# the3cloud/zktls

Hardware: AMD Instinct MI355X
Metric: trace-cells/s (higher is better)
Workload: dtype u32

## Files before the change

### zktls_amd/csrc/hash.hip

```cpp
#include "poseidon2.cuh"
#include "poseidon2_coop.cuh"
#include "kernels.h"
#include "batch.h"
#include "p24chip.h"
#include "p24chip_rows.cuh"
#include "p2chip.h"

namespace zk {

hipError_t hash_upload_p2_tables(const P2Tables& t, hipStream_t s) { return p2_upload_tables(t, s); }

__device__ __forceinline__ uint32_t load_virtual(const LeafArgs& a, uint64_t row, uint32_t vc) {
    uint32_t off = vc;
#pragma unroll
    for (int m = 0; m < MAX_LEAF_MATS; m++) {
        if (m < a.nmats) {
            if (off < a.mats[m].width) return a.mats[m].ptr[row * a.mats[m].ld + off];
            off -= a.mats[m].width;
        }
    }
    return 0u;
}

__global__ void hash_rows16_kernel(LeafArgs a, uint32_t total_w);
struct hash_rows16_kernel_bargs { LeafArgs a; uint32_t total_w; static hash_rows16_kernel_bargs make(LeafArgs a, uint32_t total_w) { return hash_rows16_kernel_bargs{a, total_w}; } };
__global__ void hash_rows16_kernel_batch(const hash_rows16_kernel_bargs* __restrict__ zk_arr);
__global__ void compress_level16_kernel(const uint32_t* __restrict__ children, uint32_t* __restrict__ parents, uint32_t count);
struct compress_level16_kernel_bargs { const uint32_t* children; uint32_t* parents; uint32_t count; static compress_level16_kernel_bargs make(const uint32_t* children, uint32_t* parents, uint32_t count) { return compress_level16_kernel_bargs{children, parents, count}; } };
__global__ void compress_level16_kernel_batch(const compress_level16_kernel_bargs* __restrict__ zk_arr);
__global__ void compress_top16_kernel(uint32_t* tree, uint32_t count);
struct compress_top16_kernel_bargs { uint32_t* tree; uint32_t count; static compress_top16_kernel_bargs make(uint32_t* tree, uint32_t count) { return compress_top16_kernel_bargs{tree, count}; } };
__global__ void compress_top16_kernel_batch(const compress_top16_kernel_bargs* __restrict__ zk_arr);
__global__ void compress_sub16_kernel(uint32_t* tree, uint32_t count, uint32_t sub);
struct compress_sub16_kernel_bargs { uint32_t* tree; uint32_t count; uint32_t sub; static compress_sub16_kernel_bargs make(uint32_t* tree, uint32_t count, uint32_t sub) { return compress_sub16_kernel_bargs{tree, count, sub}; } };
__global__ void compress_sub16_kernel_batch(const compress_sub16_kernel_bargs* __restrict__ zk_arr);
__global__ void hash_sub16_kernel(LeafArgs a, uint32_t total_w, uint32_t sub);
struct hash_sub16_kernel_bargs { LeafArgs a; uint32_t total_w; uint32_t sub; static hash_sub16_kernel_bargs make(LeafArgs a, uint32_t total_w, uint32_t sub) { return hash_sub16_kernel_bargs{a, total_w, sub}; } };
__global__ void hash_sub16_kernel_batch(const hash_sub16_kernel_bargs* __restrict__ zk_arr);

__device__ __forceinline__ void hash_rows_generic_kernel_body(const LeafArgs& a, uint32_t total_w) {
    const uint64_t row = (uint64_t)blockIdx.x * blockDim.x + threadIdx.x;
    if (row >= a.height) return;
    uint32_t s[16];
#pragma unroll
    for (int i = 0; i < 16; i++) s[i] = 0u;
    for (uint32_t q = 0; q < total_w; q += 8) {
#pragma unroll
        for (int i = 0; i < 8; i++)
            if (q + i < total_w) s[i] = load_virtual(a, row, q + i);
        p2_permute_dev(s);
    }
    uint4* d = reinterpret_cast<uint4*>(a.digests + row * 8);
    d[0] = make_uint4(s[0], s[1], s[2], s[3]);
    d[1] = make_uint4(s[4], s[5], s[6], s[7]);
}
__global__ void __launch_bounds__(256) hash_rows_generic_kernel(LeafArgs a, uint32_t total_w) { hash_rows_generic_kernel_body(a, total_w); }
struct hash_rows_generic_kernel_bargs { LeafArgs a; uint32_t total_w; static hash_rows_generic_kernel_bargs make(LeafArgs a, uint32_t total_w) { return hash_rows_generic_kernel_bargs{a, total_w}; } };
__global__ void __launch_bounds__(256) hash_rows_generic_kernel_batch(const hash_rows_generic_kernel_bargs* __restrict__ zk_arr) { const hash_rows_generic_kernel_bargs& zk_b = zk_arr[blockIdx.z]; hash_rows_generic_kernel_body(zk_b.a, zk_b.total_w); }


template <bool MX>
__device__ __forceinline__ void hash_rows_vec_body(const uint32_t* __restrict__ mat, uint64_t ld, uint32_t width, uint64_t height, uint32_t* __restrict__ digests) {
    const uint64_t row = (uint64_t)blockIdx.x * blockDim.x + threadIdx.x;
    if (MX ? row - __lane_id() >= height : row >= height) return;
    const uint4* rp = reinterpret_cast<const uint4*>(mat + (row < height ? row : height - 1) * ld);
    uint32_t s[16];
#pragma unroll
    for (int i = 0; i < 16; i++) s[i] = 0u;
    for (uint32_t q = 0; q < width / 8; q++) {
        uint4 v0 = rp[2 * q], v1 = rp[2 * q + 1];
        s[0] = v0.x; s[1] = v0.y; s[2] = v0.z; s[3] = v0.w;
        s[4] = v1.x; s[5] = v1.y; s[6] = v1.z; s[7] = v1.w;
        if (MX) p2_permute_mx_dev(s); else p2_permute_dev(s);
    }
    if (width & 4u) {
        const uint4 v0 = rp[width / 4 - 1];
        s[0] = v0.x; s[1] = v0.y; s[2] = v0.z; s[3] = v0.w;
        if (MX) p2_permute_mx_dev(s); else p2_permute_dev(s);
    }
    if (row >= height) return;
    uint4* d = reinterpret_cast<uint4*>(digests + row * 8);
    d[0] = make_uint4(s[0], s[1], s[2], s[3]);
    d[1] = make_uint4(s[4], s[5], s[6], s[7]);
}
__device__ __forceinline__ void hash_rows_vec_kernel_body(const uint32_t* __restrict__ mat, uint64_t ld, uint32_t width, uint64_t height, uint32_t* __restrict__ digests) { hash_rows_vec_body<true>(mat, ld, width, height, digests); }
__global__ void __launch_bounds__(256) __attribute__((amdgpu_waves_per_eu(5))) hash_rows_vec_kernel(const uint32_t* __restrict__ mat, uint64_t ld, uint32_t width, uint64_t height, uint32_t* __restrict__ digests) { hash_rows_vec_kernel_body(mat, ld, width, height, digests); }
struct hash_rows_vec_kernel_bargs { const uint32_t* mat; uint64_t ld; uint32_t width; uint64_t height; uint32_t* digests; static hash_rows_vec_kernel_bargs make(const uint32_t* mat, uint64_t ld, uint32_t width, uint64_t height, uint32_t* digests) { return hash_rows_vec_kernel_bargs{mat, ld, width, height, digests}; } };
__global__ void __launch_bounds__(256) __attribute__((amdgpu_waves_per_eu(5))) hash_rows_vec_kernel_batch(const hash_rows_vec_kernel_bargs* __restrict__ zk_arr) { const hash_rows_vec_kernel_bargs& zk_b = zk_arr[blockIdx.z]; hash_rows_vec_kernel_body(zk_b.mat, zk_b.ld, zk_b.width, zk_b.height, zk_b.digests); }
#ifdef ZKHIP_AB_HOOKS
__global__ void __launch_bounds__(256) hash_rows_vec_valu_kernel(const uint32_t* __restrict__ mat, uint64_t ld, uint32_t width, uint64_t height, uint32_t* __restrict__ digests) { hash_rows_vec_body<false>(mat, ld, width, height, digests); }
#endif

__device__ __forceinline__ void sponge_rows_vec(const LeafArgs& a, uint64_t row, uint32_t total_q, uint32_t s[16]) {
    int m = 0;
    uint32_t q = 0, nq = a.mats[0].width / 4;
    const uint4* rp = reinterpret_cast<const uint4*>(a.mats[0].ptr + row * a.mats[0].ld);
    for (uint32_t b = 0; b < total_q; b += 2) {
        while (q == nq) { m++; q = 0; nq = a.mats[m].width / 4; rp = reinterpret_cast<const uint4*>(a.mats[m].ptr + row * a.mats[m].ld); }
        const uint4 v0 = rp[q++];
        s[0] = v0.x; s[1] = v0.y; s[2] = v0.z; s[3] = v0.w;
        if (b + 1 < total_q) {
            while (q == nq) { m++; q = 0; nq = a.mats[m].width / 4; rp = reinterpret_cast<const uint4*>(a.mats[m].ptr + row * a.mats[m].ld); }
            const uint4 v1 = rp[q++];
            s[4] = v1.x; s[5] = v1.y; s[6] = v1.z; s[7] = v1.w;
        }
        p2_permute_dev(s);
    }
}
__device__ __forceinline__ void hash_rows_mvec_kernel_body(const LeafArgs& a, uint32_t total_q) {
    const uint64_t row = (uint64_t)blockIdx.x * blockDim.x + threadIdx.x;
    if (row >= a.height) return;
    uint32_t s[16];
#pragma unroll
    for (int i = 0; i < 16; i++) s[i] = 0u;
    sponge_rows_vec(a, row, total_q, s);
    uint4* d = reinterpret_cast<uint4*>(a.digests + row * 8);
    d[0] = make_uint4(s[0], s[1], s[2], s[3]);
    d[1] = make_uint4(s[4], s[5], s[6], s[7]);
}
__global__ void __launch_bounds__(256) hash_rows_mvec_kernel(LeafArgs a, uint32_t total_q) { hash_rows_mvec_kernel_body(a, total_q); }
struct hash_rows_mvec_kernel_bargs { LeafArgs a; uint32_t total_q; static hash_rows_mvec_kernel_bargs make(LeafArgs a, uint32_t total_q) { return hash_rows_mvec_kernel_bargs{a, total_q}; } };
__global__ void __launch_bounds__(256) hash_rows_mvec_kernel_batch(const hash_rows_mvec_kernel_bargs* __restrict__ zk_arr) { const hash_rows_mvec_kernel_bargs& zk_b = zk_arr[blockIdx.z]; hash_rows_mvec_kernel_body(zk_b.a, zk_b.total_q); }

__device__ __forceinline__ void compress_inject_mvec_kernel_body(const uint32_t* __restrict__ children, const LeafArgs& a, uint32_t total_q) {
    const uint64_t i = (uint64_t)blockIdx.x * blockDim.x + threadIdx.x;
    if (i >= a.height) return;
    const uint4* cp = reinterpret_cast<const uint4*>(children + 16 * i);
    const uint4 c0 = cp[0], c1 = cp[1], c2 = cp[2], c3 = cp[3];
    uint32_t s[16] = {c0.x, c0.y, c0.z, c0.w, c1.x, c1.y, c1.z, c1.w, c2.x, c2.y, c2.z, c2.w, c3.x, c3.y, c3.z, c3.w};
    uint32_t t[16];
#pragma unroll
    for (int k = 0; k < 16; k++) t[k] = 0u;
    p2_permute_dev(s);
    sponge_rows_vec(a, i, total_q, t);
#pragma unroll
    for (int k = 0; k < 8; k++) s[8 + k] = t[k];
    p2_permute_dev(s);
    uint4* d = reinterpret_cast<uint4*>(a.digests + i * 8);
    d[0] = make_uint4(s[0], s[1], s[2], s[3]);
    d[1] = make_uint4(s[4], s[5], s[6], s[7]);
}
__global__ void __launch_bounds__(256) compress_inject_mvec_kernel(const uint32_t* __restrict__ children, LeafArgs a, uint32_t total_q) { compress_inject_mvec_kernel_body(children, a, total_q); }
struct compress_inject_mvec_kernel_bargs { const uint32_t* children; LeafArgs a; uint32_t total_q; static compress_inject_mvec_kernel_bargs make(const uint32_t* children, LeafArgs a, uint32_t total_q) { return compress_inject_mvec_kernel_bargs{children, a, total_q}; } };
__global__ void __launch_bounds__(256) compress_inject_mvec_kernel_batch(const compress_inject_mvec_kernel_bargs* __restrict__ zk_arr) { const compress_inject_mvec_kernel_bargs& zk_b = zk_arr[blockIdx.z]; compress_inject_mvec_kernel_body(zk_b.children, zk_b.a, zk_b.total_q); }

static bool leaf_mats_vec(const LeafArgs& a) {
    for (int m = 0; m < a.nmats; m++) {
        const MatDesc& d = a.mats[m];
        if (d.width == 0 || d.width % 4 || d.ld % 4 || (reinterpret_cast<uintptr_t>(d.ptr) & 15)) return false;
    }
    return a.nmats >= 1;
}
hipError_t launch_compress_inject(const uint32_t* children, const LeafArgs& a, hipStream_t s) {
    if (a.height == 0) return hipSuccess;
    if (a.nmats < 1 || a.nmats > MAX_LEAF_MATS || !leaf_mats_vec(a)) return hipErrorInvalidValue;
    uint32_t total = 0;
    for (int m = 0; m < a.nmats; m++) total += a.mats[m].width;
    ZK_LAUNCH(compress_inject_mvec_kernel, compress_inject_mvec_kernel_batch, compress_inject_mvec_kernel_bargs, dim3((unsigned)((a.height + 255) / 256)), dim3(256), 0, s, children, a, total / 4);
    return hipGetLastError();
}
bool compress_inject_ok(const LeafArgs& a) { return a.height > coop_max_nodes() && leaf_mats_vec(a); }

hipError_t launch_hash_rows(const LeafArgs& a, hipStream_t s) {
    if (a.height == 0) return hipSuccess;
    if (a.nmats < 1 || a.nmats > MAX_LEAF_MATS) return hipErrorInvalidValue;
    uint32_t total = 0;
    for (int m = 0; m < a.nmats; m++) total += a.mats[m].width;
    if (a.height <= coop_max_nodes()) {
        const uint64_t threads = a.height * 16;
        ZK_LAUNCH(hash_rows16_kernel, hash_rows16_kernel_batch, hash_rows16_kernel_bargs, dim3((unsigned)((threads + 255) / 256)), dim3(256), 0, s, a, total);
        return hipGetLastError();
    }
    dim3 block(256), grid((unsigned)((a.height + 255) / 256));
    const MatDesc& m0 = a.mats[0];
    bool vec = a.nmats == 1 && m0.width % 4 == 0 && m0.ld % 4 == 0 &&
               (reinterpret_cast<uintptr_t>(m0.ptr) & 15) == 0;
#ifdef ZKHIP_AB_HOOKS
    static const bool valu = getenv("ZKHIP_HASH_VEC_VALU") != nullptr;
    if (vec && valu) {
        hash_rows_vec_valu_kernel<<<grid, block, 0, s>>>(m0.ptr, m0.ld, m0.width, a.height, a.digests);
        return hipGetLastError();
    }
#endif
    if (vec)
        ZK_LAUNCH(hash_rows_vec_kernel, hash_rows_vec_kernel_batch, hash_rows_vec_kernel_bargs, grid, block, 0, s, m0.ptr, m0.ld, m0.width, a.height, a.digests);
    else if (leaf_mats_vec(a))
        ZK_LAUNCH(hash_rows_mvec_kernel, hash_rows_mvec_kernel_batch, hash_rows_mvec_kernel_bargs, grid, block, 0, s, a, total / 4);
    else
        ZK_LAUNCH(hash_rows_generic_kernel, hash_rows_generic_kernel_batch, hash_rows_generic_kernel_bargs, grid, block, 0, s, a, total);
    return hipGetLastError();
}

__device__ __forceinline__ void compress_node(const uint32_t* children, uint32_t* parent) {
    const uint4* cp = reinterpret_cast<const uint4*>(children);
    uint4 v0 = cp[0], v1 = cp[1], v2 = cp[2], v3 = cp[3];
    uint32_t s[16] = {v0.x, v0.y, v0.z, v0.w, v1.x, v1.y, v1.z, v1.w,
                      v2.x, v2.y, v2.z, v2.w, v3.x, v3.y, v3.z, v3.w};
    p2_permute_dev(s);
    uint4* d = reinterpret_cast<uint4*>(parent);
    d[0] = make_uint4(s[0], s[1], s[2], s[3]);
    d[1] = make_uint4(s[4], s[5], s[6], s[7]);
}

__device__ __forceinline__ void compress_level_kernel_body(const uint32_t* __restrict__ children, uint32_t* __restrict__ parents, uint64_t count) {
    const uint64_t i = (uint64_t)blockIdx.x * blockDim.x + threadIdx.x;
    if (i >= count) return;
    compress_node(children + 16 * i, parents + 8 * i);
}
__global__ void __launch_bounds__(256) compress_level_kernel(const uint32_t* __restrict__ children, uint32_t* __restrict__ parents, uint64_t count) { compress_level_kernel_body(children, parents, count); }
struct compress_level_kernel_bargs { const uint32_t* children; uint32_t* parents; uint64_t count; static compress_level_kernel_bargs make(const uint32_t* children, uint32_t* parents, uint64_t count) { return compress_level_kernel_bargs{children, parents, count}; } };
__global__ void __launch_bounds__(256) compress_level_kernel_batch(const compress_level_kernel_bargs* __restrict__ zk_arr) { const compress_level_kernel_bargs& zk_b = zk_arr[blockIdx.z]; compress_level_kernel_body(zk_b.children, zk_b.parents, zk_b.count); }

hipError_t launch_compress_level(const uint32_t* children, uint32_t* parents, uint64_t count, hipStream_t s) {
    if (count == 0) return hipSuccess;
    if (count <= coop_max_nodes()) {
        const uint64_t threads = count * 16;
        ZK_LAUNCH(compress_level16_kernel, compress_level16_kernel_batch, compress_level16_kernel_bargs, dim3((unsigned)((threads + 255) / 256)), dim3(256), 0, s, children, parents, (uint32_t)count);
        return hipGetLastError();
    }
    ZK_LAUNCH(compress_level_kernel, compress_level_kernel_batch, compress_level_kernel_bargs, dim3((unsigned)((count + 255) / 256)), dim3(256), 0, s, children, parents, count);
    return hipGetLastError();
}

__device__ __forceinline__ void inject_kernel_body(uint32_t* __restrict__ nodes, const uint32_t* __restrict__ extra, uint64_t count) {
    const uint64_t i = (uint64_t)blockIdx.x * blockDim.x + threadIdx.x;
    if (i >= count) return;
    const uint4* a = reinterpret_cast<const uint4*>(nodes + 8 * i);
    const uint4* b = reinterpret_cast<const uint4*>(extra + 8 * i);
    const uint4 v0 = a[0], v1 = a[1], v2 = b[0], v3 = b[1];
    uint32_t s[16] = {v0.x, v0.y, v0.z, v0.w, v1.x, v1.y, v1.z, v1.w, v2.x, v2.y, v2.z, v2.w, v3.x, v3.y, v3.z, v3.w};
    p2_permute_dev(s);
    uint4* d = reinterpret_cast<uint4*>(nodes + 8 * i);
    d[0] = make_uint4(s[0], s[1], s[2], s[3]);
    d[1] = make_uint4(s[4], s[5], s[6], s[7]);
}
__global__ void __launch_bounds__(256) inject_kernel(uint32_t* __restrict__ nodes, const uint32_t* __restrict__ extra, uint64_t count) { inject_kernel_body(nodes, extra, count); }
struct inject_kernel_bargs { uint32_t* nodes; const uint32_t* extra; uint64_t count; static inject_kernel_bargs make(uint32_t* nodes, const uint32_t* extra, uint64_t count) { return inject_kernel_bargs{nodes, extra, count}; } };
__global__ void __launch_bounds__(256) inject_kernel_batch(const inject_kernel_bargs* __restrict__ zk_arr) { const inject_kernel_bargs& zk_b = zk_arr[blockIdx.z]; inject_kernel_body(zk_b.nodes, zk_b.extra, zk_b.count); }

hipError_t launch_inject(uint32_t* nodes, const uint32_t* extra, uint64_t count, hipStream_t s) {
    if (count == 0) return hipSuccess;
    ZK_LAUNCH(inject_kernel, inject_kernel_batch, inject_kernel_bargs, dim3((unsigned)((count + 255) / 256)), dim3(256), 0, s, nodes, extra, count);
    return hipGetLastError();
}

__device__ __forceinline__ void compress_top_kernel_body(uint32_t* tree, uint32_t count) {
    uint32_t* level = tree;
    for (uint32_t n = count; n > 1; n >>= 1) {
        uint32_t* next = level + 8 * (size_t)n;
        for (uint32_t i = threadIdx.x; i < n / 2; i += blockDim.x) compress_node(level + 16 * (size_t)i, next + 8 * (size_t)i);
        __threadfence_block();
        __syncthreads();
        level = next;
    }
}
__global__ void __launch_bounds__(1024) compress_top_kernel(uint32_t* tree, uint32_t count) { compress_top_kernel_body(tree, count); }
struct compress_top_kernel_bargs { uint32_t* tree; uint32_t count; static compress_top_kernel_bargs make(uint32_t* tree, uint32_t count) { return compress_top_kernel_bargs{tree, count}; } };
__global__ void __launch_bounds__(1024) compress_top_kernel_batch(const compress_top_kernel_bargs* __restrict__ zk_arr) { const compress_top_kernel_bargs& zk_b = zk_arr[blockIdx.z]; compress_top_kernel_body(zk_b.tree, zk_b.count); }

hipError_t launch_compress_top(uint32_t* tree, uint32_t count, hipStream_t s) {
    if (count <= 1) return hipSuccess;
    if (count > COOP_TOP_NODES) return hipErrorInvalidValue;
    unsigned threads = count * 8 < 64 ? 64 : (count * 8 > 1024 ? 1024 : count * 8);
// ... 957 lines not shown
```

### zktls_amd/csrc/poseidon2.cuh

```cuda
#pragma once
#include "babybear.cuh"
#include "p2_params.h"

namespace zk {

struct P2Consts {
    uint32_t ext_rc[8][16];
    uint32_t int_rc[13];
    uint32_t diag[16];
    uint32_t ext_rcm[8][16];
    uint32_t int_rcm[13];
};
struct P2Raw {
    uint32_t ext16[8][16], int16[13], diag16[16];
    uint32_t ext24[8][24], int24[21], diag24[24];
};
constexpr P2Consts make_p2_consts(const P2Raw& raw) {
    P2Consts k{};
    for (int r = 0; r < 8; r++)
        for (int i = 0; i < 16; i++) k.ext_rc[r][i] = to_monty(raw.ext16[r][i]);
    for (int r = 0; r < 13; r++) k.int_rc[r] = to_monty(raw.int16[r]);
    for (int i = 0; i < 16; i++) k.diag[i] = to_monty(raw.diag16[i]);
    for (int r = 0; r < 8; r++)
        for (int i = 0; i < 16; i++) k.ext_rcm[r][i] = k.ext_rc[r][i] - P;
// ... 33 lines not shown
}

ZK_HD constexpr void p2_external_linear(uint32_t s[16]) {
    p2_m4(s[0], s[1], s[2], s[3]);
    p2_m4(s[4], s[5], s[6], s[7]);
    p2_m4(s[8], s[9], s[10], s[11]);
    p2_m4(s[12], s[13], s[14], s[15]);
    uint32_t t0 = fadd(fadd(s[0], s[4]), fadd(s[8], s[12]));
    uint32_t t1 = fadd(fadd(s[1], s[5]), fadd(s[9], s[13]));
    uint32_t t2 = fadd(fadd(s[2], s[6]), fadd(s[10], s[14]));
    uint32_t t3 = fadd(fadd(s[3], s[7]), fadd(s[11], s[15]));
#if defined(__HIP_DEVICE_COMPILE__)
#pragma unroll
#endif
    for (int b = 0; b < 16; b += 4) {
        s[b] = fadd(s[b], t0);
        s[b + 1] = fadd(s[b + 1], t1);
        s[b + 2] = fadd(s[b + 2], t2);
        s[b + 3] = fadd(s[b + 3], t3);
    }
}

struct Mat4 { uint32_t m[4][4]; };
template <bool HL>
constexpr Mat4 m4_matrix() {
    Mat4 a{};
    for (int j = 0; j < 4; j++) {
        uint32_t e[4] = {0, 0, 0, 0};
        e[j] = MONTY_R1;
        if (HL) p2_m4_hl(e[0], e[1], e[2], e[3]); else p2_m4(e[0], e[1], e[2], e[3]);
        for (int i = 0; i < 4; i++) a.m[i][j] = e[i];
    }
    return a;
}
constexpr Mat4 mat4_inverse(Mat4 a) {
    Mat4 b{};
    for (int i = 0; i < 4; i++) b.m[i][i] = MONTY_R1;
    for (int c = 0; c < 4; c++) {
        int piv = c;
        while (a.m[piv][c] == 0) piv++;
        for (int j = 0; j < 4; j++) {
            uint32_t t = a.m[c][j]; a.m[c][j] = a.m[piv][j]; a.m[piv][j] = t;
            t = b.m[c][j]; b.m[c][j] = b.m[piv][j]; b.m[piv][j] = t;
        }
        const uint32_t inv = finv(a.m[c][c]);
        for (int j = 0; j < 4; j++) { a.m[c][j] = fmul(a.m[c][j], inv); b.m[c][j] = fmul(b.m[c][j], inv); }
        for (int r = 0; r < 4; r++) {
            if (r == c) continue;
            const uint32_t f = a.m[r][c];
            for (int j = 0; j < 4; j++) {
                a.m[r][j] = fsub(a.m[r][j], fmul(f, a.m[c][j]));
                b.m[r][j] = fsub(b.m[r][j], fmul(f, b.m[c][j]));
            }
        }
    }
    return b;
}
template <int W, bool HL>
constexpr void external_preimage(const uint32_t v[W], uint32_t out[W]) {
    const Mat4 inv4 = mat4_inverse(m4_matrix<HL>());
    uint32_t sum[4] = {0, 0, 0, 0};
    for (int b = 0; b < W; b += 4)
        for (int i = 0; i < 4; i++) {
            uint32_t acc = 0;
            for (int j = 0; j < 4; j++) acc = fadd(acc, fmul(inv4.m[i][j], v[b + j]));
            out[b + i] = acc;
            sum[i] = fadd(sum[i], acc);
        }
    const uint32_t f = finv(to_monty(W / 4 + 1));
    for (int b = 0; b < W; b += 4)
        for (int i = 0; i < 4; i++) out[b + i] = fsub(out[b + i], fmul(f, sum[i]));
}


struct P2IntConsts { int32_t diag[16]; int32_t rc_fold[13]; int32_t k_sum; };
struct P2PairConsts { int32_t rs_mul[16]; int32_t d2[16]; int32_t e[16]; int32_t k_sum_a, k_sum_b, c15, pair; };
constexpr int P2_PAIR_SHIFT = 24;
struct P2ExtFold { int64_t c[8][16]; };
struct P24Consts { uint32_t ext_rc[8][24]; uint32_t int_rc[21]; uint32_t diag[24]; uint32_t ext_rcm[8][24]; uint32_t int_rcm[21]; };
struct P24IntConsts { int32_t diag[24]; int32_t rc_fold[21]; int32_t k_sum; };
struct P24ExtFold { int64_t c[8][24]; };
constexpr uint32_t MX_BIAS = 0x80808080u - P;
constexpr int mx_elem(int g, int q) { return (q & 3) + 4 * g + 8 * (q >> 2); }
struct alignas(16) P2MxConsts { int64_t fold[8][2][8]; uint32_t in0[2][8]; };
struct P2Tables {
    P2Consts k16; P2IntConsts ik16; P2PairConsts pk16; P2ExtFold ef16;
    P24Consts k24; P24IntConsts ik24; P24ExtFold ef24;
    P2MxConsts mx16;
};
constexpr P2IntConsts make_p2_int_consts(const P2Raw& raw) {
    P2IntConsts k{};
    for (int i = 0; i < 16; i++) k.diag[i] = centered(to_monty(raw.diag16[i]));
    for (int r = 0; r + 1 < 13; r++) k.rc_fold[r] = centered(to_monty(to_monty(raw.int16[r + 1])));
    k.rc_fold[12] = 0;
    k.k_sum = centered(to_monty(32u));
    return k;
}
struct P2Bound { uint64_t v; bool ok; };
constexpr P2Bound p2_bound_red(uint64_t x, bool ok) {
    if (!ok || x > 0x7FFFFFFFFFFFFFFFull - ((uint64_t)P << 31)) return P2Bound{0, false};
    const uint64_t r = (x >> 32) + P / 2 + 1;
    return P2Bound{r, r <= 0x7FFFFFFFull};
}
constexpr P2Bound p2_bound_sbox(uint64_t t, bool ok) {
    const P2Bound x2 = p2_bound_red(t * t, ok && t <= 0x7FFFFFFFull);
    const P2Bound x4 = p2_bound_red(x2.v * x2.v, x2.ok);
    const P2Bound x6 = p2_bound_red(x4.v * x2.v, x4.ok);
    return p2_bound_red(x6.v * t, x6.ok);
}
constexpr bool p2_pair_budget_ok(uint64_t sum_d, int sh) {
    const uint64_t H = (P - 1) / 2;
    if (sum_d > ((uint64_t)1 << 24)) return false;
    uint64_t b0 = P, bv = P;
    {
        const P2Bound u = p2_bound_sbox(b0, true);
        const P2Bound s = p2_bound_red((u.v + 15 * bv) << 27, u.ok);
        const P2Bound n0 = p2_bound_red(u.v * H + s.v * H + H, s.ok), nv = p2_bound_red(bv * H + s.v * H, s.ok);
        if (!n0.ok || !nv.ok || n0.v > P - 1 || nv.v > P - 1) return false;
        b0 = n0.v; bv = nv.v;
    }
    for (int k = 0; k < 6; k++) {
        const P2Bound u = p2_bound_sbox(b0, true);
        const P2Bound st = p2_bound_red((u.v + 15 * bv) << sh, u.ok);
        const P2Bound v0 = p2_bound_red(u.v * H + st.v * H + H, st.ok);
        const P2Bound u2 = p2_bound_sbox(v0.v, v0.ok);
        const P2Bound s1 = p2_bound_red(sum_d * bv + st.v * (15ull << (32 - sh)) + u2.v, u2.ok);
        const P2Bound n0 = p2_bound_red(u2.v * H + s1.v * H + H, s1.ok), nv = p2_bound_red(bv * H + st.v * H + s1.v * H, s1.ok);
        if (!n0.ok || !nv.ok || n0.v > P - 1 || nv.v > P - 1 || v0.v > P - 1) return false;
        b0 = n0.v; bv = nv.v;
    }
    return true;
}
static_assert(p2_pair_budget_ok(49151, P2_PAIR_SHIFT) && p2_pair_budget_ok(15u << 15, P2_PAIR_SHIFT) && !p2_pair_budget_ok(49151, 27),
              "paired partial rounds: the range budget");
constexpr bool p2_pair_diag_ok(const P2Raw& raw) {
    uint64_t sum_d = 0;
    for (int i = 1; i < 16; i++) {
        if (raw.diag16[i] < 1 || raw.diag16[i] > (1u << 15)) return false;
        sum_d += raw.diag16[i];
    }
    return p2_pair_budget_ok(sum_d, P2_PAIR_SHIFT);
}
constexpr uint32_t p2_pow2_mod(int k) {
    uint32_t x = 1;
    for (int i = 0; i < k; i++) x = fdbl(x);
    return x;
}
constexpr P2PairConsts make_p2_pair_consts(const P2Raw& raw) {
    P2PairConsts k{};
    const uint32_t ka = p2_pow2_mod(64 - P2_PAIR_SHIFT);
    for (int i = 0; i < 16; i++) {
        const uint32_t d = raw.diag16[i] % P, dm = to_monty(d);
        k.rs_mul[i] = i == 0 ? 1 : (int32_t)(d <= (1u << 15) ? d : 0);
        k.d2[i] = centered(fmul(dm, dm));
        k.e[i] = centered((uint32_t)((uint64_t)d * ka % P));
    }
    k.k_sum_a = centered(ka);
    k.k_sum_b = centered(to_monty(to_monty(1u)));
    k.c15 = (int32_t)(15u << (32 - P2_PAIR_SHIFT));
    k.pair = p2_pair_diag_ok(raw) ? 1 : 0;
    return k;
}
constexpr P2ExtFold make_p2_ext_fold(const P2Consts& k16) {
    P2ExtFold k{};
    for (int r = 0; r < 8; r++) {
        uint32_t v[16] = {}, u[16] = {};
        if (r == 3) v[0] = k16.int_rc[0];
        else if (r < 7) for (int i = 0; i < 16; i++) v[i] = k16.ext_rc[r + 1][i];
        external_preimage<16, false>(v, u);
        for (int i = 0; i < 16; i++) k.c[r][i] = (int64_t)centered(to_monty(u[i])) + ((int64_t)P << 31);
    }
    return k;
}
constexpr P24Consts make_p24_consts(const P2Raw& raw) {
    P24Consts k{};
    for (int r = 0; r < 8; r++)
        for (int i = 0; i < 24; i++) k.ext_rc[r][i] = to_monty(raw.ext24[r][i]);
    for (int r = 0; r < 21; r++) k.int_rc[r] = to_monty(raw.int24[r]);
    for (int i = 0; i < 24; i++) k.diag[i] = to_monty(raw.diag24[i]);
    for (int r = 0; r < 8; r++)
        for (int i = 0; i < 24; i++) k.ext_rcm[r][i] = k.ext_rc[r][i] - P;
    for (int r = 0; r < 21; r++) k.int_rcm[r] = k.int_rc[r] - P;
    return k;
}
constexpr P24IntConsts make_p24_int_consts(const P2Raw& raw) {
    P24IntConsts k{};
    for (int i = 0; i < 24; i++) k.diag[i] = centered(to_monty(raw.diag24[i]));
    for (int r = 0; r + 1 < 21; r++) k.rc_fold[r] = centered(to_monty(to_monty(raw.int24[r + 1])));
    k.rc_fold[20] = 0;
    k.k_sum = centered(to_monty(64u));
    return k;
}
constexpr void p24_external_linear_ce(uint32_t s[24]) {
    for (int b = 0; b < 24; b += 4) p2_m4_hl(s[b], s[b + 1], s[b + 2], s[b + 3]);
    uint32_t t[4] = {0, 0, 0, 0};
    for (int k = 0; k < 4; k++)
        for (int b = 0; b < 24; b += 4) t[k] = fadd(t[k], s[b + k]);
    for (int i = 0; i < 24; i++) s[i] = fadd(s[i], t[i & 3]);
}
constexpr P24ExtFold make_p24_ext_fold(const P24Consts& k24) {
    P24ExtFold k{};
    for (int r = 0; r < 8; r++) {
        uint32_t v[24] = {}, u[24] = {};
        if (r == 3) v[0] = k24.int_rc[0];
        else if (r < 7) for (int i = 0; i < 24; i++) v[i] = k24.ext_rc[r + 1][i];
        external_preimage<24, true>(v, u);
        for (int i = 0; i < 24; i++) k.c[r][i] = (int64_t)centered(to_monty(u[i])) + ((int64_t)P << 31);
    }
    return k;
}
constexpr P2MxConsts make_p2_mx_consts(const P2Consts& k16, const P2ExtFold& ef16) {
    P2MxConsts k{};
    uint32_t u0[16] = {};
    external_preimage<16, false>(k16.ext_rc[0], u0);
    for (int g = 0; g < 2; g++)
        for (int q = 0; q < 8; q++) {
            for (int r = 0; r < 8; r++) k.fold[r][g][q] = ef16.c[r][mx_elem(g, q)] + ((int64_t)MX_BIAS << 32);
            k.in0[g][q] = u0[mx_elem(g, q)] + MX_BIAS;
        }
    return k;
}
constexpr P2Tables derive_tables(const P2Raw& raw) {
    P2Tables t{};
    t.k16 = make_p2_consts(raw); t.ik16 = make_p2_int_consts(raw); t.pk16 = make_p2_pair_consts(raw); t.ef16 = make_p2_ext_fold(t.k16);
    t.k24 = make_p24_consts(raw); t.ik24 = make_p24_int_consts(raw); t.ef24 = make_p24_ext_fold(t.k24);
    t.mx16 = make_p2_mx_consts(t.k16, t.ef16);
    return t;
}
constexpr bool tables_ok(const P2Raw& raw, const P2Tables& t) {
    for (int r = 0; r < 8; r++) for (int i = 0; i < 16; i++) if (raw.ext16[r][i] >= P) return false;
    for (int r = 0; r < 13; r++) if (raw.int16[r] >= P) return false;
    for (int i = 0; i < 16; i++) if (raw.diag16[i] >= P) return false;
    for (int r = 0; r < 8; r++) for (int i = 0; i < 24; i++) if (raw.ext24[r][i] >= P) return false;
    for (int r = 0; r < 21; r++) if (raw.int24[r] >= P) return false;
    for (int i = 0; i < 24; i++) if (raw.diag24[i] >= P) return false;
    for (int r = 0; r < 7; r++) {
        uint32_t v[16] = {}, u[16] = {};
        if (r == 3) v[0] = t.k16.int_rc[0];
        else for (int i = 0; i < 16; i++) v[i] = t.k16.ext_rc[r + 1][i];
        external_preimage<16, false>(v, u);
        p2_external_linear(u);
        for (int i = 0; i < 16; i++) if (u[i] != v[i]) return false;
        uint32_t v2[24] = {}, u2[24] = {};
        if (r == 3) v2[0] = t.k24.int_rc[0];
        else for (int i = 0; i < 24; i++) v2[i] = t.k24.ext_rc[r + 1][i];
        external_preimage<24, true>(v2, u2);
        p24_external_linear_ce(u2);
        for (int i = 0; i < 24; i++) if (u2[i] != v2[i]) return false;
    }
    for (int g = 0; g < 2; g++)
        for (int q = 0; q < 8; q++) {
            if (t.mx16.in0[g][q] - MX_BIAS >= P) return false;
            uint32_t v[16] = {}, u[16] = {};
            for (int i = 0; i < 16; i++) v[i] = t.k16.ext_rc[0][i];
            external_preimage<16, false>(v, u);
            if (t.mx16.in0[g][q] - MX_BIAS != u[mx_elem(g, q)]) return false;
            for (int r = 0; r < 8; r++) {
                const int64_t c = t.mx16.fold[r][g][q] - ((int64_t)MX_BIAS << 32) - ((int64_t)P << 31);
                if (c != t.ef16.c[r][mx_elem(g, q)] - ((int64_t)P << 31) || c < -(int64_t)(P / 2) || c > (int64_t)(P / 2)) return false;
            }
        }
    if ((t.pk16.pair != 0) != p2_pair_diag_ok(raw) || (t.pk16.pair != 0 && t.pk16.pair != 1)) return false;
    if (t.pk16.pair) {
        const uint32_t r2 = to_monty(to_monty(1u));
        const auto canon = [](int32_t x) { return x < 0 ? (uint32_t)(x + (int32_t)P) : (uint32_t)x; };
        const auto small = [](int32_t x) { return x >= -(int32_t)(P / 2) && x <= (int32_t)(P / 2); };
        if (canon(t.pk16.k_sum_b) != r2 || !small(t.pk16.k_sum_a) || !small(t.pk16.k_sum_b)) return false;
        if ((uint32_t)((uint64_t)canon(t.pk16.k_sum_a) * (1u << P2_PAIR_SHIFT) % P) != r2) return false;
        if (t.pk16.c15 != (int32_t)(15u << (32 - P2_PAIR_SHIFT)) || t.pk16.rs_mul[0] != 1) return false;
        for (int i = 1; i < 16; i++) {
            const uint32_t d = raw.diag16[i];
            if (t.pk16.rs_mul[i] != (int32_t)d || !small(t.pk16.d2[i]) || !small(t.pk16.e[i])) return false;
            if (canon(t.pk16.d2[i]) != (uint32_t)((uint64_t)d * d % P * to_monty(1u) % P)) return false;
            if (canon(t.pk16.e[i]) != (uint32_t)((uint64_t)d * canon(t.pk16.k_sum_a) % P)) return false;
        }
    }
    return true;
}
constexpr P2Raw builtin_raw() {
    P2Raw raw{};
    for (int r = 0; r < 8; r++) for (int i = 0; i < 16; i++) raw.ext16[r][i] = P2_EXTERNAL_RC[r][i];
    for (int r = 0; r < 13; r++) raw.int16[r] = P2_INTERNAL_RC[r];
    for (int i = 0; i < 16; i++) raw.diag16[i] = P2_INTERNAL_DIAG[i];
    for (int r = 0; r < 8; r++) for (int i = 0; i < 24; i++) raw.ext24[r][i] = P24_EXTERNAL_RC[r][i];
    for (int r = 0; r < 21; r++) raw.int24[r] = P24_INTERNAL_RC[r];
    for (int i = 0; i < 24; i++) raw.diag24[i] = P24_INTERNAL_DIAG[i];
    return raw;
}
constexpr P2Raw P2_BUILTIN_RAW = builtin_raw();
constexpr P2Tables P2_BUILTIN = derive_tables(P2_BUILTIN_RAW);
static_assert(tables_ok(P2_BUILTIN_RAW, P2_BUILTIN), "M_E (M_E^-1 rc) != rc");
static_assert(P2_BUILTIN.pk16.pair == 1, "the built-in diagonal takes the paired partial rounds");

extern P2Tables g_p2_tables;
#if defined(__HIPCC__)
static __constant__ P2Tables d_p2_tables = P2_BUILTIN;
static inline hipError_t p2_upload_tables(const P2Tables& host, hipStream_t s) {
    return hipMemcpyToSymbolAsync(HIP_SYMBOL(d_p2_tables), &host, sizeof(P2Tables), 0, hipMemcpyHostToDevice, s);
}
#endif
#if defined(__HIP_DEVICE_COMPILE__)
#define P2T d_p2_tables
#else
#define P2T g_p2_tables
#endif
#define P2K (P2T.k16)
#define P2IK (P2T.ik16)
#define P2PK (P2T.pk16)
#define P2EF (P2T.ef16)
#define P24K (P2T.k24)
#define P24IK (P2T.ik24)
#define P24EF (P2T.ef24)
#define P24HK (P2T.k24)

ZK_HD void p2_internal_linear(uint32_t s[16]) {
    uint32_t a = fadd(fadd(s[0], s[1]), fadd(s[2], s[3]));
    uint32_t b = fadd(fadd(s[4], s[5]), fadd(s[6], s[7]));
    uint32_t c = fadd(fadd(s[8], s[9]), fadd(s[10], s[11]));
    uint32_t d = fadd(fadd(s[12], s[13]), fadd(s[14], s[15]));
    uint32_t sum = fadd(fadd(a, b), fadd(c, d));
#if defined(__HIP_DEVICE_COMPILE__)
#pragma unroll
#endif
    for (int i = 0; i < 16; i++) s[i] = fadd(fmul(s[i], P2K.diag[i]), sum);
}

ZK_HD void p2_permute_scalar(uint32_t s[16]) {
    p2_external_linear(s);
#if defined(__HIP_DEVICE_COMPILE__)
#pragma unroll 1
#endif
    for (int r = 0; r < 4; r++) {
#if defined(__HIP_DEVICE_COMPILE__)
#pragma unroll
#endif
        for (int i = 0; i < 16; i++) s[i] = p2_sbox(fadd(s[i], P2K.ext_rc[r][i]));
        p2_external_linear(s);
    }
#if defined(__HIP_DEVICE_COMPILE__)
#pragma unroll 1
#endif
    for (int r = 0; r < 13; r++) {
        s[0] = p2_sbox(fadd(s[0], P2K.int_rc[r]));
        p2_internal_linear(s);
// ... 117 lines not shown
    asm volatile("s_mov_b32 %0, 0x1000000" : "=s"(sh24));
    p2_internal_round_dev(v, 0, sh);
    if (P2PK.pair) {
#pragma unroll P2_INT_UNROLL
        for (int r = 1; r < 13; r += 2) p2_internal_pair_dev(v, r, sh24);
    } else {
#pragma unroll P2_INT_UNROLL
        for (int r = 1; r < 13; r++) p2_internal_round_dev(v, r, sh);
    }
#pragma unroll
    for (int i = 0; i < 16; i++) s[i] = dcanon(v[i]);
}
ZK_D uint32_t p2_sbox_fold_dev(int32_t t, int64_t fold_biased) {
    const int32_t x2 = dsmont(t, t);
    const int32_t x4 = dsmont(x2, x2);
    const int32_t x6 = dsmont(x4, x2);
    return dred(dmred_lazy((uint64_t)dsmac(x6, t, fold_biased)));
}
ZK_D void p2_external_linear_signed_dev(uint32_t s[16]) {
    p2_m4_dev(s[0], s[1], s[2], s[3]);
    p2_m4_dev(s[4], s[5], s[6], s[7]);
    p2_m4_dev(s[8], s[9], s[10], s[11]);
    p2_m4_dev(s[12], s[13], s[14], s[15]);
    const uint32_t t0 = dadd(dadd(s[0], s[4]), dadd(s[8], s[12])) - P;
    const uint32_t t1 = dadd(dadd(s[1], s[5]), dadd(s[9], s[13])) - P;
    const uint32_t t2 = dadd(dadd(s[2], s[6]), dadd(s[10], s[14])) - P;
    const uint32_t t3 = dadd(dadd(s[3], s[7]), dadd(s[11], s[15])) - P;
#pragma unroll
    for (int b = 0; b < 16; b += 4) {
        s[b] += t0;
        s[b + 1] += t1;
        s[b + 2] += t2;
        s[b + 3] += t3;
    }
}
ZK_D void p2_permute_dev(uint32_t s[16]) {
    p2_external_linear_dev(s);
#pragma unroll
    for (int i = 0; i < 16; i++) s[i] += P2K.ext_rcm[0][i];
#pragma unroll 1
    for (int r = 0; r < 4; r++) {
#pragma unroll
        for (int i = 0; i < 16; i++) s[i] = p2_sbox_fold_dev((int32_t)s[i], P2EF.c[r][i]);
        p2_external_linear_signed_dev(s);
    }
    p2_internal_rounds_dev(s);
#pragma unroll
    for (int i = 0; i < 16; i++) s[i] += P2K.ext_rcm[4][i];
#pragma unroll 1
    for (int r = 4; r < 8; r++) {
#pragma unroll
        for (int i = 0; i < 16; i++) s[i] = p2_sbox_fold_dev((int32_t)s[i], P2EF.c[r][i]);
        p2_external_linear_signed_dev(s);
    }
#pragma unroll
    for (int i = 0; i < 16; i++) s[i] = dcanon((int32_t)s[i]);
}

typedef int p2mx_v4i __attribute__((ext_vector_type(4)));
typedef int p2mx_v16i __attribute__((ext_vector_type(16)));
constexpr int32_t MX_C24 = centered((uint32_t)(((uint64_t)1 << 56) % P));
constexpr uint32_t p2_me_entry(int i, int j) {
    return ((i >> 2) == (j >> 2) ? 2u : 1u) * (uint32_t)(0x1132u >> (4 * ((j - i) & 3)) & 15u);
}
constexpr uint32_t p2_mx_a_word(int lane, int idx) {
    const int m = lane & 31, h = lane >> 5, mb = idx >> 3, kb = (idx >> 2) & 1, r = idx & 3;
    return p2_me_entry(mx_elem((m >> 2) & 1, 4 * mb + (m >> 3)), mx_elem(h, 4 * kb + r)) << (8 * (m & 3));
}
struct P2MxA { uint32_t w[64][16]; };
constexpr P2MxA make_p2_mx_a() {
    P2MxA a{};
    for (int l = 0; l < 64; l++)
        for (int i = 0; i < 16; i++) a.w[l][i] = p2_mx_a_word(l, i);
    return a;
}
static_assert(p2_me_entry(0, 0) == 4 && p2_me_entry(0, 1) == 6 && p2_me_entry(1, 0) == 2 && p2_me_entry(3, 0) == 6 && p2_me_entry(4, 1) == 3,
              "M_E entries");
static __constant__ P2MxA d_p2_mx_a = make_p2_mx_a();
ZK_D void p2_mx_load_a(p2mx_v4i a[4]) {
    const uint4* p = reinterpret_cast<const uint4*>(d_p2_mx_a.w[__lane_id()]);
#pragma unroll
    for (int i = 0; i < 4; i++) { const uint4 v = p[i]; a[i] = p2mx_v4i{(int)v.x, (int)v.y, (int)v.z, (int)v.w}; }
}
ZK_D void p2_mx_layer(const uint32_t d[8], const p2mx_v4i a[4], int32_t w[8]) {
    const p2mx_v4i b0 = {(int)d[0], (int)d[1], (int)d[2], (int)d[3]}, b1 = {(int)d[4], (int)d[5], (int)d[6], (int)d[7]};
#pragma unroll
    for (int mb = 0; mb < 2; mb++) {
        p2mx_v16i y = {};
        y = __builtin_amdgcn_mfma_i32_32x32x32_i8(a[2 * mb], b0, y, 0, 0, 0);
        y = __builtin_amdgcn_mfma_i32_32x32x32_i8(a[2 * mb + 1], b1, y, 0, 0, 0);
#pragma unroll
        for (int e = 0; e < 4; e++) {
            const uint32_t L = (uint32_t)y[4 * e] + ((uint32_t)y[4 * e + 1] << 8) + ((uint32_t)y[4 * e + 2] << 16);
            w[4 * mb + e] = dsmred((int64_t)((uint64_t)L << 32) + (int64_t)y[4 * e + 3] * MX_C24);
        }
    }
}
ZK_D uint32_t p2_sbox_mx_dev(int32_t t, int64_t fold_mx) {
    const int32_t x2 = dsmont(t, t);
    const int32_t x4 = dsmont(x2, x2);
    const int32_t x6 = dsmont(x4, x2);
    return dmred_lazy((uint64_t)dsmac(x6, t, fold_mx)) ^ 0x80808080u;
}
ZK_D void p2_mx_swap(uint32_t x[8], uint32_t y[8]) {
#pragma unroll
    for (int q = 0; q < 8; q++) {
        const auto r = __builtin_amdgcn_permlane32_swap(x[q], y[q], false, false);
        x[q] = r[0]; y[q] = r[1];
    }
}
ZK_D void p2_mx_full_rounds(int32_t wa[8], int32_t wb[8], int r0, int h) {
    p2mx_v4i a[4];
    p2_mx_load_a(a);
#pragma unroll 1
    for (int r = r0; r < r0 + 4; r++) {
        const int64_t* f = P2T.mx16.fold[r][h];
        uint32_t d[8];
#pragma unroll
        for (int q = 0; q < 8; q++) d[q] = p2_sbox_mx_dev(wa[q], f[q]);
        p2_mx_layer(d, a, wa);
#pragma unroll
        for (int q = 0; q < 8; q++) d[q] = p2_sbox_mx_dev(wb[q], f[q]);
        p2_mx_layer(d, a, wb);
    }
}
ZK_D void p2_permute_mx_dev(uint32_t s[16]) {
    const int h = __lane_id() >> 5;
    uint32_t x[8], y[8];
    int32_t wa[8], wb[8];
#pragma unroll
    for (int q = 0; q < 8; q++) { x[q] = s[mx_elem(0, q)]; y[q] = s[mx_elem(1, q)]; }
    p2_mx_swap(x, y);
    {
        const uint32_t* c = P2T.mx16.in0[h];
        uint32_t da[8], db[8];
        p2mx_v4i a[4];
        p2_mx_load_a(a);
#pragma unroll
        for (int q = 0; q < 8; q++) { da[q] = (x[q] + c[q]) ^ 0x80808080u; db[q] = (y[q] + c[q]) ^ 0x80808080u; }
        p2_mx_layer(da, a, wa);
        p2_mx_layer(db, a, wb);
    }
    p2_mx_full_rounds(wa, wb, 0, h);
#pragma unroll
    for (int q = 0; q < 8; q++) { x[q] = (uint32_t)wa[q]; y[q] = (uint32_t)wb[q]; }
    p2_mx_swap(x, y);
#pragma unroll
    for (int q = 0; q < 8; q++) { s[mx_elem(0, q)] = x[q]; s[mx_elem(1, q)] = y[q]; }
    p2_internal_rounds_dev(s);
#pragma unroll
    for (int q = 0; q < 8; q++) { x[q] = s[mx_elem(0, q)] + P2K.ext_rcm[4][mx_elem(0, q)]; y[q] = s[mx_elem(1, q)] + P2K.ext_rcm[4][mx_elem(1, q)]; }
    p2_mx_swap(x, y);
#pragma unroll
    for (int q = 0; q < 8; q++) { wa[q] = (int32_t)x[q]; wb[q] = (int32_t)y[q]; }
    p2_mx_full_rounds(wa, wb, 4, h);
#pragma unroll
    for (int q = 0; q < 8; q++) { x[q] = dcanon(wa[q]); y[q] = dcanon(wb[q]); }
    p2_mx_swap(x, y);
#pragma unroll
    for (int q = 0; q < 8; q++) { s[mx_elem(0, q)] = x[q]; s[mx_elem(1, q)] = y[q]; }
}
#endif

#if defined(__HIPCC__)
ZK_D void p24_external_linear_dev(uint32_t s[24]) {
#pragma unroll
    for (int b = 0; b < 24; b += 4) p2_m4_hl_dev(s[b], s[b + 1], s[b + 2], s[b + 3]);
    uint32_t t[4];
#pragma unroll
    for (int k = 0; k < 4; k++)
        t[k] = dadd(dadd(dadd(s[k], s[4 + k]), dadd(s[8 + k], s[12 + k])), dadd(s[16 + k], s[20 + k]));
#pragma unroll
    for (int i = 0; i < 24; i++) s[i] = dadd(s[i], t[i & 3]);
}
ZK_D void p24_internal_rounds_dev(uint32_t s[24]) {
    int32_t v[24];
#pragma unroll
    for (int i = 0; i < 24; i++) v[i] = (int32_t)s[i];
    int32_t sh;
    asm volatile("s_mov_b32 %0, 0x4000000" : "=s"(sh));
#pragma unroll P2_INT_UNROLL
    for (int r = 0; r < 21; r++) {
        v[0] = p2_sbox_signed(v[0]);
        int64_t T = 0;
#pragma unroll
        for (int j = 0; j < 24; j++) T = dsmac_uniform(v[j], sh, T);
        const int32_t sum = dsmred(T);
        int64_t T2 = dsmac_s(sum, P24IK.k_sum, 0);
        v[0] = dsmred(dsmac_s(v[0], P24IK.diag[0], T2 + (int64_t)P24IK.rc_fold[r]));
#pragma unroll
        for (int i = 1; i < 24; i++) v[i] = dsmred(dsmac_s(v[i], P24IK.diag[i], T2));
    }
#pragma unroll
    for (int i = 0; i < 24; i++) s[i] = dcanon(v[i]);
}
ZK_D void p24_external_linear_signed_dev(uint32_t s[24]) {
#pragma unroll
    for (int b = 0; b < 24; b += 4) p2_m4_hl_dev(s[b], s[b + 1], s[b + 2], s[b + 3]);
    uint32_t t[4];
#pragma unroll
    for (int k = 0; k < 4; k++)
        t[k] = dadd(dadd(dadd(s[k], s[4 + k]), dadd(s[8 + k], s[12 + k])), dadd(s[16 + k], s[20 + k])) - P;
#pragma unroll
    for (int i = 0; i < 24; i++) s[i] += t[i & 3];
}
ZK_D void p24_permute_dev(uint32_t s[24]) {
    p24_external_linear_dev(s);
#pragma unroll
    for (int i = 0; i < 24; i++) s[i] += P24K.ext_rcm[0][i];
#pragma unroll 1
    for (int r = 0; r < 4; r++) {
#pragma unroll
        for (int i = 0; i < 24; i++) s[i] = p2_sbox_fold_dev((int32_t)s[i], P24EF.c[r][i]);
        p24_external_linear_signed_dev(s);
    }
    p24_internal_rounds_dev(s);
#pragma unroll
    for (int i = 0; i < 24; i++) s[i] += P24K.ext_rcm[4][i];
#pragma unroll 1
    for (int r = 4; r < 8; r++) {
#pragma unroll
        for (int i = 0; i < 24; i++) s[i] = p2_sbox_fold_dev((int32_t)s[i], P24EF.c[r][i]);
        p24_external_linear_signed_dev(s);
    }
#pragma unroll
    for (int i = 0; i < 24; i++) s[i] = dcanon((int32_t)s[i]);
}
#endif

inline void p24_external_linear(uint32_t s[24]) {
    for (int b = 0; b < 24; b += 4) p2_m4_hl(s[b], s[b + 1], s[b + 2], s[b + 3]);
    uint32_t t[4];
    for (int k = 0; k < 4; k++) {
        t[k] = 0;
        for (int b = 0; b < 24; b += 4) t[k] = fadd(t[k], s[b + k]);
    }
    for (int i = 0; i < 24; i++) s[i] = fadd(s[i], t[i & 3]);
}
inline void p24_permute(uint32_t s[24]) {
    p24_external_linear(s);
    for (int r = 0; r < 4; r++) {
        for (int i = 0; i < 24; i++) s[i] = p2_sbox(fadd(s[i], P24HK.ext_rc[r][i]));
        p24_external_linear(s);
    }
// ... 21 lines not shown
```

Before: 20.35 billion.

## Specialize MFMA Poseidon2 sponge permutations by absorb/squeeze form to skip unused work

Replaces the row-hashing sponge kernel with a variant that keeps the capacity in a transformed basis between absorbs. The first external layer's round constants are folded into precomputed capacity and last-round constants. In the final round only the MFMA output blocks that are actually needed are computed (rate or capacity half), which cuts MFMA and reduction work per permutation. This adds new constexpr-derived tables with validation checks, but makes the sponge more intricate and dependent on algebraic identities holding.

```diff
diff --git a/zktls_amd/csrc/hash.hip b/zktls_amd/csrc/hash.hip
--- a/zktls_amd/csrc/hash.hip
+++ b/zktls_amd/csrc/hash.hip
@@ -83,12 +83,49 @@
     d[0] = make_uint4(s[0], s[1], s[2], s[3]);
     d[1] = make_uint4(s[4], s[5], s[6], s[7]);
 }
-__device__ __forceinline__ void hash_rows_vec_kernel_body(const uint32_t* __restrict__ mat, uint64_t ld, uint32_t width, uint64_t height, uint32_t* __restrict__ digests) { hash_rows_vec_body<true>(mat, ld, width, height, digests); }
+__device__ __forceinline__ void hash_rows_sponge_body(const uint32_t* __restrict__ mat, uint64_t ld, uint32_t width, uint64_t height, uint32_t* __restrict__ digests) {
+    const uint64_t row = (uint64_t)blockIdx.x * blockDim.x + threadIdx.x;
+    if (row - __lane_id() >= height) return;
+    const uint4* rp = reinterpret_cast<const uint4*>(mat + (row < height ? row : height - 1) * ld);
+    uint32_t s[16];
+#pragma unroll
+    for (int i = 0; i < 8; i++) { s[i] = 0u; s[8 + i] = (uint32_t)P2T.mx16.cap0[i]; }
+    const uint32_t nb = width / 8, half = width & 4u;
+    uint32_t q = 0;
+    for (; q + 1 < nb; q++) {
+        const uint4 v0 = rp[2 * q], v1 = rp[2 * q + 1];
+        s[0] = v0.x; s[1] = v0.y; s[2] = v0.z; s[3] = v0.w;
+        s[4] = v1.x; s[5] = v1.y; s[6] = v1.z; s[7] = v1.w;
+        p2_permute_mx_form<P2MxForm::ABSORB>(s);
+    }
+    if (half && nb) {
+        const uint4 v0 = rp[2 * q], v1 = rp[2 * q + 1];
+        s[0] = v0.x; s[1] = v0.y; s[2] = v0.z; s[3] = v0.w;
+        s[4] = v1.x; s[5] = v1.y; s[6] = v1.z; s[7] = v1.w;
+        p2_permute_mx_form<P2MxForm::ABSORB_RATE>(s);
+        q++;
+    }
+    if (width) {
+        const uint4 v0 = rp[2 * q];
+        s[0] = v0.x; s[1] = v0.y; s[2] = v0.z; s[3] = v0.w;
+        if (!half) {
+            const uint4 v1 = rp[2 * q + 1];
+            s[4] = v1.x; s[5] = v1.y; s[6] = v1.z; s[7] = v1.w;
+        }
+        p2_permute_mx_form<P2MxForm::SQUEEZE>(s);
+    }
+    if (row >= height) return;
+    uint4* d = reinterpret_cast<uint4*>(digests + row * 8);
+    d[0] = make_uint4(s[0], s[1], s[2], s[3]);
+    d[1] = make_uint4(s[4], s[5], s[6], s[7]);
+}
+__device__ __forceinline__ void hash_rows_vec_kernel_body(const uint32_t* __restrict__ mat, uint64_t ld, uint32_t width, uint64_t height, uint32_t* __restrict__ digests) { hash_rows_sponge_body(mat, ld, width, height, digests); }
 __global__ void __launch_bounds__(256) __attribute__((amdgpu_waves_per_eu(5))) hash_rows_vec_kernel(const uint32_t* __restrict__ mat, uint64_t ld, uint32_t width, uint64_t height, uint32_t* __restrict__ digests) { hash_rows_vec_kernel_body(mat, ld, width, height, digests); }
 struct hash_rows_vec_kernel_bargs { const uint32_t* mat; uint64_t ld; uint32_t width; uint64_t height; uint32_t* digests; static hash_rows_vec_kernel_bargs make(const uint32_t* mat, uint64_t ld, uint32_t width, uint64_t height, uint32_t* digests) { return hash_rows_vec_kernel_bargs{mat, ld, width, height, digests}; } };
 __global__ void __launch_bounds__(256) __attribute__((amdgpu_waves_per_eu(5))) hash_rows_vec_kernel_batch(const hash_rows_vec_kernel_bargs* __restrict__ zk_arr) { const hash_rows_vec_kernel_bargs& zk_b = zk_arr[blockIdx.z]; hash_rows_vec_kernel_body(zk_b.mat, zk_b.ld, zk_b.width, zk_b.height, zk_b.digests); }
 #ifdef ZKHIP_AB_HOOKS
 __global__ void __launch_bounds__(256) hash_rows_vec_valu_kernel(const uint32_t* __restrict__ mat, uint64_t ld, uint32_t width, uint64_t height, uint32_t* __restrict__ digests) { hash_rows_vec_body<false>(mat, ld, width, height, digests); }
+__global__ void __launch_bounds__(256) __attribute__((amdgpu_waves_per_eu(5))) hash_rows_vec_closed_kernel(const uint32_t* __restrict__ mat, uint64_t ld, uint32_t width, uint64_t height, uint32_t* __restrict__ digests) { hash_rows_vec_body<true>(mat, ld, width, height, digests); }
 #endif
 
 __device__ __forceinline__ void sponge_rows_vec(const LeafArgs& a, uint64_t row, uint32_t total_q, uint32_t s[16]) {
@@ -179,6 +216,11 @@
     static const bool valu = getenv("ZKHIP_HASH_VEC_VALU") != nullptr;
     if (vec && valu) {
         hash_rows_vec_valu_kernel<<<grid, block, 0, s>>>(m0.ptr, m0.ld, m0.width, a.height, a.digests);
+        return hipGetLastError();
+    }
+    static const bool closed = getenv("ZKHIP_HASH_VEC_CLOSED") != nullptr;
+    if (vec && closed) {
+        hash_rows_vec_closed_kernel<<<grid, block, 0, s>>>(m0.ptr, m0.ld, m0.width, a.height, a.digests);
         return hipGetLastError();
     }
 #endif
diff --git a/zktls_amd/csrc/poseidon2.cuh b/zktls_amd/csrc/poseidon2.cuh
--- a/zktls_amd/csrc/poseidon2.cuh
+++ b/zktls_amd/csrc/poseidon2.cuh
@@ -139,7 +139,7 @@
 struct P24ExtFold { int64_t c[8][24]; };
 constexpr uint32_t MX_BIAS = 0x80808080u - P;
 constexpr int mx_elem(int g, int q) { return (q & 3) + 4 * g + 8 * (q >> 2); }
-struct alignas(16) P2MxConsts { int64_t fold[8][2][8]; uint32_t in0[2][8]; };
+struct alignas(16) P2MxConsts { int64_t fold[8][2][8]; uint32_t in0[2][8]; int64_t fold7a[2][8]; int32_t cap0[8]; };
 struct P2Tables {
     P2Consts k16; P2IntConsts ik16; P2PairConsts pk16; P2ExtFold ef16;
     P24Consts k24; P24IntConsts ik24; P24ExtFold ef24;
@@ -275,6 +275,11 @@
             for (int r = 0; r < 8; r++) k.fold[r][g][q] = ef16.c[r][mx_elem(g, q)] + ((int64_t)MX_BIAS << 32);
             k.in0[g][q] = u0[mx_elem(g, q)] + MX_BIAS;
         }
+    uint32_t v[16] = {}, u[16] = {};
+    for (int i = 8; i < 16; i++) { v[i] = u0[i]; k.cap0[i - 8] = centered(u0[i]); }
+    external_preimage<16, false>(v, u);
+    for (int g = 0; g < 2; g++)
+        for (int q = 0; q < 8; q++) k.fold7a[g][q] = (int64_t)centered(to_monty(u[mx_elem(g, q)])) + ((int64_t)P << 31) + ((int64_t)MX_BIAS << 32);
     return k;
 }
 constexpr P2Tables derive_tables(const P2Raw& raw) {
@@ -317,6 +322,24 @@
                 if (c != t.ef16.c[r][mx_elem(g, q)] - ((int64_t)P << 31) || c < -(int64_t)(P / 2) || c > (int64_t)(P / 2)) return false;
             }
         }
+    {
+        uint32_t v[16] = {}, u[16] = {}, w[16] = {};
+        for (int i = 0; i < 16; i++) v[i] = t.k16.ext_rc[0][i];
+        external_preimage<16, false>(v, u);
+        for (int i = 0; i < 16; i++) v[i] = i < 8 ? 0u : u[i];
+        external_preimage<16, false>(v, w);
+        for (int g = 0; g < 2; g++)
+            for (int q = 0; q < 8; q++) {
+                const int64_t c = t.mx16.fold7a[g][q] - ((int64_t)MX_BIAS << 32) - ((int64_t)P << 31);
+                if (c != (int64_t)centered(to_monty(w[mx_elem(g, q)])) || c < -(int64_t)(P / 2) || c > (int64_t)(P / 2)) return false;
+            }
+        p2_external_linear(w);
+        for (int i = 0; i < 16; i++) if (w[i] != v[i]) return false;
+        for (int i = 0; i < 8; i++) {
+            const int32_t c = t.mx16.cap0[i];
+            if (c < -(int32_t)(P / 2) || c > (int32_t)(P / 2) || (c < 0 ? (uint32_t)(c + (int32_t)P) : (uint32_t)c) != u[8 + i]) return false;
+        }
+    }
     if ((t.pk16.pair != 0) != p2_pair_diag_ok(raw) || (t.pk16.pair != 0 && t.pk16.pair != 1)) return false;
     if (t.pk16.pair) {
         const uint32_t r2 = to_monty(to_monty(1u));
@@ -600,19 +623,20 @@
 #pragma unroll
     for (int i = 0; i < 4; i++) { const uint4 v = p[i]; a[i] = p2mx_v4i{(int)v.x, (int)v.y, (int)v.z, (int)v.w}; }
 }
+ZK_D void p2_mx_layer_block(const uint32_t d[8], const p2mx_v4i a[4], int32_t w[8], int mb) {
+    const p2mx_v4i b0 = {(int)d[0], (int)d[1], (int)d[2], (int)d[3]}, b1 = {(int)d[4], (int)d[5], (int)d[6], (int)d[7]};
+    p2mx_v16i y = {};
+    y = __builtin_amdgcn_mfma_i32_32x32x32_i8(a[2 * mb], b0, y, 0, 0, 0);
+    y = __builtin_amdgcn_mfma_i32_32x32x32_i8(a[2 * mb + 1], b1, y, 0, 0, 0);
+#pragma unroll
+    for (int e = 0; e < 4; e++) {
+        const uint32_t L = (uint32_t)y[4 * e] + ((uint32_t)y[4 * e + 1] << 8) + ((uint32_t)y[4 * e + 2] << 16);
+        w[4 * mb + e] = dsmred((int64_t)((uint64_t)L << 32) + (int64_t)y[4 * e + 3] * MX_C24);
+    }
+}
 ZK_D void p2_mx_layer(const uint32_t d[8], const p2mx_v4i a[4], int32_t w[8]) {
-    const p2mx_v4i b0 = {(int)d[0], (int)d[1], (int)d[2], (int)d[3]}, b1 = {(int)d[4], (int)d[5], (int)d[6], (int)d[7]};
-#pragma unroll
-    for (int mb = 0; mb < 2; mb++) {
-        p2mx_v16i y = {};
-        y = __builtin_amdgcn_mfma_i32_32x32x32_i8(a[2 * mb], b0, y, 0, 0, 0);
-        y = __builtin_amdgcn_mfma_i32_32x32x32_i8(a[2 * mb + 1], b1, y, 0, 0, 0);
-#pragma unroll
-        for (int e = 0; e < 4; e++) {
-            const uint32_t L = (uint32_t)y[4 * e] + ((uint32_t)y[4 * e + 1] << 8) + ((uint32_t)y[4 * e + 2] << 16);
-            w[4 * mb + e] = dsmred((int64_t)((uint64_t)L << 32) + (int64_t)y[4 * e + 3] * MX_C24);
-        }
-    }
+    p2_mx_layer_block(d, a, w, 0);
+    p2_mx_layer_block(d, a, w, 1);
 }
 ZK_D uint32_t p2_sbox_mx_dev(int32_t t, int64_t fold_mx) {
     const int32_t x2 = dsmont(t, t);
@@ -642,7 +666,34 @@
         p2_mx_layer(d, a, wb);
     }
 }
-ZK_D void p2_permute_mx_dev(uint32_t s[16]) {
+template <int BLOCKS>
+ZK_D void p2_mx_last_rounds(int32_t wa[8], int32_t wb[8], int h, const int64_t* f7) {
+    p2mx_v4i a[4];
+    p2_mx_load_a(a);
+    uint32_t d[8];
+#pragma unroll 1
+    for (int r = 4; r < 7; r++) {
+        const int64_t* f = P2T.mx16.fold[r][h];
+#pragma unroll
+        for (int q = 0; q < 8; q++) d[q] = p2_sbox_mx_dev(wa[q], f[q]);
+        p2_mx_layer(d, a, wa);
+#pragma unroll
+        for (int q = 0; q < 8; q++) d[q] = p2_sbox_mx_dev(wb[q], f[q]);
+        p2_mx_layer(d, a, wb);
+    }
+#pragma unroll
+    for (int q = 0; q < 8; q++) d[q] = p2_sbox_mx_dev(wa[q], f7[q]);
+    if (BLOCKS & 1) p2_mx_layer_block(d, a, wa, 0);
+    if (BLOCKS & 2) p2_mx_layer_block(d, a, wa, 1);
+#pragma unroll
+    for (int q = 0; q < 8; q++) d[q] = p2_sbox_mx_dev(wb[q], f7[q]);
+    if (BLOCKS & 1) p2_mx_layer_block(d, a, wb, 0);
+    if (BLOCKS & 2) p2_mx_layer_block(d, a, wb, 1);
+}
+enum class P2MxForm { CLOSED, ABSORB, ABSORB_RATE, SQUEEZE };
+template <P2MxForm F>
+ZK_D void p2_permute_mx_form(uint32_t s[16]) {
+    constexpr bool SPONGE = F != P2MxForm::CLOSED;
     const int h = __lane_id() >> 5;
     uint32_t x[8], y[8];
     int32_t wa[8], wb[8];
@@ -655,7 +706,10 @@
         p2mx_v4i a[4];
         p2_mx_load_a(a);
 #pragma unroll
-        for (int q = 0; q < 8; q++) { da[q] = (x[q] + c[q]) ^ 0x80808080u; db[q] = (y[q] + c[q]) ^ 0x80808080u; }
+        for (int q = 0; q < 8; q++) {
+            const uint32_t cq = SPONGE && q >= 4 ? 0x80808080u : c[q];
+            da[q] = (x[q] + cq) ^ 0x80808080u; db[q] = (y[q] + cq) ^ 0x80808080u;
+        }
         p2_mx_layer(da, a, wa);
         p2_mx_layer(db, a, wb);
     }
@@ -671,13 +725,30 @@
     p2_mx_swap(x, y);
 #pragma unroll
     for (int q = 0; q < 8; q++) { wa[q] = (int32_t)x[q]; wb[q] = (int32_t)y[q]; }
-    p2_mx_full_rounds(wa, wb, 4, h);
-#pragma unroll
-    for (int q = 0; q < 8; q++) { x[q] = dcanon(wa[q]); y[q] = dcanon(wb[q]); }
-    p2_mx_swap(x, y);
-#pragma unroll
-    for (int q = 0; q < 8; q++) { s[mx_elem(0, q)] = x[q]; s[mx_elem(1, q)] = y[q]; }
-}
+    if (!SPONGE) {
+        p2_mx_full_rounds(wa, wb, 4, h);
+#pragma unroll
+        for (int q = 0; q < 8; q++) { x[q] = dcanon(wa[q]); y[q] = dcanon(wb[q]); }
+        p2_mx_swap(x, y);
+#pragma unroll
+        for (int q = 0; q < 8; q++) { s[mx_elem(0, q)] = x[q]; s[mx_elem(1, q)] = y[q]; }
+    } else {
+        constexpr int BLOCKS = F == P2MxForm::SQUEEZE ? 1 : F == P2MxForm::ABSORB ? 2 : 3;
+        p2_mx_last_rounds<BLOCKS>(wa, wb, h, F == P2MxForm::SQUEEZE ? P2T.mx16.fold[7][h] : P2T.mx16.fold7a[h]);
+#pragma unroll
+        for (int q = 0; q < 8; q++) {
+            if (!(BLOCKS >> (q >> 2) & 1)) continue;
+            const uint32_t xa = q < 4 ? dcanon(wa[q]) : (uint32_t)wa[q], yb = q < 4 ? dcanon(wb[q]) : (uint32_t)wb[q];
+            const auto r = __builtin_amdgcn_permlane32_swap(xa, yb, false, false);
+            s[mx_elem(0, q)] = r[0]; s[mx_elem(1, q)] = r[1];
+        }
+        if (F == P2MxForm::ABSORB) {
+#pragma unroll
+            for (int i = 0; i < 8; i++) s[i] = 0u;
+        }
+    }
+}
+ZK_D void p2_permute_mx_dev(uint32_t s[16]) { p2_permute_mx_form<P2MxForm::CLOSED>(s); }
 #endif
 
 #if defined(__HIPCC__)
```

New measurement: 20.73 billion (median of 6 runs). +1.9%, better.
